# parklab/Salamander

Measured on AMD Instinct MI355X. Metric: KL-NMF update-steps/sec (96xN, k=50), higher is better.
Workload: dtype f64; 1 GPU; c2: KLNMF n_signatures=50 on synthetic Poisson counts 96x100000 per GPU (joint update_WH steps, device resident); n_features=96, n_samples_per_gpu=100000, n_samples_total=100000, n_signatures=50, parallelism=single GPU

## Files before the change

salamander_amd/csrc/salnmf_fused_kernel.h:

```cpp
#pragma once
#include "salnmf_kernels.h"

namespace salnmf {

constexpr int FK_NSEC = 16;
template <int KS, int KTM, int KR, bool DO_G, bool DO_U, bool DO_STATS, bool WTS = false, bool PERSIST = false, bool BLOCKED = false, bool RGIVEN = false,
          bool MVJ = false>
__global__ void __launch_bounds__(BLOCK, 1) fused_kernel(FusedParams p) {
#ifdef SALNMF_DEV_PROFILE
    unsigned long long tks[FK_NSEC] = {0, 0, 0, 0, 0, 0, 0, 0, 0, 0, 0, 0, 0, 0, 0, 0}, tk0 = __builtin_amdgcn_s_memtime(), tk1, ntl = 0;
#define FK_TICK(i) do { __builtin_amdgcn_sched_barrier(0); tk1 = __builtin_amdgcn_s_memtime(); tks[i] += tk1 - tk0; tk0 = tk1; __builtin_amdgcn_sched_barrier(0); } while (0)
#else
#define FK_TICK(i) do { } while (0)
#endif
    static_assert(!MVJ || (DO_G && DO_U && DO_STATS && !WTS && !PERSIST && !BLOCKED && !RGIVEN), "MVJ: the unweighted MvNMF pass pair");
    static_assert(!RGIVEN || (WTS && !DO_STATS && !PERSIST), "given ratio: the weighted-capable plain passes only (with BLOCKED: the update_H pass of one feature block)");
    static_assert(!PERSIST || (DO_G && DO_U && !DO_STATS && !WTS), "the persistent mode is the plain joint step");
    static_assert(!BLOCKED || (DO_U && !DO_STATS && WTS && !PERSIST), "feature blocks: the weighted-capable update_H pass, alone or with the block's numerator");
    using G_ = Geo<KS>;
    constexpr int KT = KTM;
    constexpr int KP = G_::KP, LS = G_::LS, HV = G_::HV;
    constexpr int KB = 16 * KTM;
    constexpr int NVP = KR == 0 ? 0 : (KR == 1 ? 4 : (KR == 2 ? 8 : 16));
    static_assert(KR >= 0 && KR <= 4 && KB + KR <= KP, "remainder columns must fit the padded layout");
    constexpr int WROWS = 4 * KS > 16 * KTM + KR ? 4 * KS : 16 * KTM + KR;
    static_assert(WROWS <= G_::WROWS, "never more rows than the padded layout");
    constexpr bool HDMA_FITS = (WROWS * WS + WAVES * (2 * G_::HL + G_::RL) + KP + (DO_STATS ? LOGTAB_DOUBLES : 0) + (WTS ? WAVES * 32 : 0)) * 8 <= 160 * 1024;
    constexpr bool HDMA = DO_G && DO_U && !PERSIST && !BLOCKED && !RGIVEN && !MVJ && HDMA_FITS;
    constexpr int REGION = (HDMA ? 2 : 1) * G_::HL + G_::RL;
    constexpr int LDSD = WROWS * WS + WAVES * REGION;
    constexpr int LDS_EXTRA = KP + (DO_STATS ? LOGTAB_DOUBLES : 0) + (WTS ? WAVES * 32 : 0);
    using CO_ = EpiGeo<KT, KR, 160 * 1024 / 8 - LDS_EXTRA>;
    constexpr int LDS_MAIN = LDSD > CO_::need(CO_::ROUNDS) ? LDSD : CO_::need(CO_::ROUNDS);
    __shared__ __attribute__((aligned(16))) double lds[LDS_MAIN + LDS_EXTRA];

    constexpr bool MVU = DO_U && DO_STATS && (!DO_G || MVJ);
    if (DO_STATS && p.skip_flag != nullptr && __hip_atomic_load((gsync_t*)p.skip_flag, __ATOMIC_RELAXED, __HIP_MEMORY_SCOPE_AGENT) != 0u) return;
    const int nwg = (int)gridDim.x - ((MVU && p.sideW != nullptr) ? 1 : 0);
    if (MVU && p.sideW != nullptr && (int)blockIdx.x == nwg) {
        static_assert(!MVU || KP * (MV_WS + 2 * MV_LD + 1) + 1 <= LDSD, "the W-only algebra must fit this geometry's LDS");
        const int K = p.K;
        double* Wl = lds;
        double* S = Wl + K * MV_WS;
        double* T = S + K * MV_LD;
        mv_prepare_W_body<BLOCK>(p.sideW, K, p.V, p.sideDelta, p.sideA, p.sideB, p.sideLogdet, Wl, S, T, T + K * MV_LD);
        return;
    }
    const int nsteps = PERSIST ? p.nsteps : 1;
    for (int step = 0; step < nsteps; ++step) {
    int tid = threadIdx.x;
    if (PERSIST) asm volatile("" : "+v"(tid));
    const int lane = tid & 63;
    const int wave = tid >> 6;
    const int c16 = lane & 15;
    const int q = lane >> 4;
    const int V = p.V, K = p.K;
    const int64_t N = p.N;
    const double* __restrict__ const wkl = WTS ? p.wkl : nullptr;
    const double* __restrict__ const wlh = WTS ? p.wlh : nullptr;

    double* Wl = lds;
    double* Hl = lds + WROWS * WS + wave * REGION;
    double* const Rl = lds + WROWS * WS + wave * REGION + G_::HL;
    double* Hnx = Hl + (HDMA ? G_::HL + G_::RL : 0);
    double* const Hdma0 = lds + WROWS * WS + __builtin_amdgcn_readfirstlane(wave) * REGION;
    int hsel = 0;

    double* hsl = lds + LDS_MAIN;
    if (p.hscale && tid < KP) hsl[tid] = p.hscale[tid];
    double* ltab = hsl + KP;
    if (DO_STATS) stage_logtab(ltab, tid);
    double* wgt = ltab + (DO_STATS ? LOGTAB_DOUBLES : 0) + wave * 32;

    d4 g[KT][VT];
    double grem[KR > 0 ? KR : 1][VT];
    double hsum[KT > 0 ? KT : 1];
    double hsum_rem = 0.0;
    double klacc = 0.0;
    double klacc_b = 0.0;
    if (MVU) {
#pragma unroll
        for (int kt = 0; kt < KT; ++kt) hsum[kt] = 0.0;
    }

    const int64_t tstride = (int64_t)(MVU ? nwg : (int)gridDim.x) * WAVES;
    int64_t tile = 0;
    constexpr bool COOP = DO_G && DO_U && !RGIVEN && !MVJ && !BLOCKED;
    constexpr int CSLAB = WROWS * WS + REGION;
    static_assert(!COOP || CO_::COOP_DOUBLES <= (WAVES - 1) * REGION, "the cooperative tile's numerator park must fit the idle waves' LDS");
    const int64_t nleft = p.ntiles % tstride;
    const bool coop = COOP && nleft > 0 && nleft <= (int64_t)gridDim.x && p.hscale == nullptr;
    const int64_t nfull = coop ? p.ntiles - nleft : p.ntiles;

    int hrow[HV], hcol[HV];
#pragma unroll
    for (int j = 0; j < HV; ++j) {
        int e = 2 * lane + 128 * j;
        hrow[j] = e / KP;
        hcol[j] = e - hrow[j] * KP;
    }

    d2 hpre[HV];
    double x[VT][4];
    d2 wpre = (d2){1.0, 0.0};

    constexpr int HPR = LS / 2, HNI = (16 * HPR + 63) / 64;
    int hoff[HDMA ? HNI : 1];
    if (HDMA) {
#pragma unroll
        for (int i = 0; i < HNI; ++i) {
            const int sp = 64 * i + lane, row = sp / HPR, c = sp - row * HPR;
            hoff[i] = row < 16 ? row * KP + 2 * (c < HPR - 1 ? c : HPR - 2) : -1;
        }
    }
    auto load_tile_H = [&](int64_t t) __attribute__((always_inline)) {
        const int64_t n0 = t * 16;
        if constexpr (HDMA) {
            const double* hsrc = p.H + n0 * KP;
            const unsigned m0base = (unsigned)(size_t)(__attribute__((address_space(3))) void*)(Hdma0 + hsel * (G_::HL + G_::RL));
#pragma unroll
            for (int i = 0; i < HNI; ++i)
                if (64 * (i + 1) <= 16 * HPR || hoff[i] >= 0)
                    asm volatile("s_mov_b32 m0, %1\n\ts_nop 0\n\tglobal_load_lds_dwordx4 %0, off"
                                 :
                                 : "v"(hsrc + hoff[i]), "s"(__builtin_amdgcn_readfirstlane(m0base + 1024u * i))
                                 : "memory");
            hsel ^= 1;
        } else {
            const d2* hsrc = reinterpret_cast<const d2*>(p.H + n0 * KP) + lane;
#pragma unroll
            for (int j = 0; j < HV; ++j) hpre[j] = hsrc[64 * j];
        }
    };
    auto load_tile_X = [&](int64_t t) __attribute__((always_inline)) {
        const int64_t n0 = t * 16;
        const double* xsrc = p.X + (n0 + q) * VMAX + c16;
#pragma unroll
        for (int vt = 0; vt < VT; ++vt)
#pragma unroll
            for (int r = 0; r < 4; ++r) x[vt][r] = xsrc[4 * r * VMAX + 16 * vt];
        if (WTS) {
            wpre[0] = p.wkl_eff[n0 + c16];
            wpre[1] = p.wlh_eff[n0 + c16];
        }
    };
    auto load_tile = [&](int64_t t) __attribute__((always_inline)) {
        load_tile_H(t);
        load_tile_X(t);
    };
    bool x_first = false;
    const bool coop_here = COOP && HDMA && coop && (int64_t)blockIdx.x < nleft;
    bool coop_fetched = false;
    auto coop_prefetch = [&]() __attribute__((always_inline)) {
        const int64_t ct = nfull + blockIdx.x;
        const int wvu = __builtin_amdgcn_readfirstlane(wave);
        if (wvu == 0) load_tile_H(ct);
        const int vt0 = wvu < 2 ? 2 * wvu : wvu + 2, nvt = wvu < 2 ? 2 : 1;
        const double* xsrc = p.X + (ct * 16 + q) * VMAX + c16;
#pragma unroll
        for (int i = 0; i < 2; ++i)
#pragma unroll
            for (int r = 0; r < 4; ++r) x[i][r] = xsrc[4 * r * VMAX + 16 * (vt0 + (i < nvt ? i : 0))];
        coop_fetched = true;
    };

    auto process_half = [&](int64_t tile, auto halftag) __attribute__((always_inline)) {
        constexpr int HALF = decltype(halftag)::value;
        constexpr bool TG = DO_G && HALF != 1, TU = DO_U && HALF != 2;
        const int64_t n0 = tile * 16;
        if (WTS) *reinterpret_cast<d2*>(wgt + 2 * c16) = wpre;
        if (!HDMA && HALF != 2 && p.hscale) {
#pragma unroll
            for (int j = 0; j < HV; ++j) {
                hpre[j][0] = clip_lo(hpre[j][0] * hsl[hcol[j]], kEps);
                hpre[j][1] = clip_lo(hpre[j][1] * hsl[hcol[j] + 1], kEps);
            }
        }
        if (!HDMA && HALF != 2) {
#pragma unroll
            for (int j = 0; j < HV; ++j) {
                *reinterpret_cast<d2*>(Hl + hrow[j] * LS + hcol[j]) = hpre[j];
            }
        }
        if (HDMA) {
            static_assert(VT * 4 == 24, "the X tile is 24 loads per lane");
            if (x_first) asm volatile("s_waitcnt vmcnt(0)" ::: "memory");
            else asm volatile("s_waitcnt vmcnt(24)" ::: "memory");
            x_first = false;
        }
        __builtin_amdgcn_wave_barrier();
        d4 uacc0[BLOCKED ? KT : 1];
        if (BLOCKED && TU) {
            const double* ua = p.Uacc + (n0 + q) * KP + c16;
#pragma unroll
            for (int kt = 0; kt < KT; ++kt)
#pragma unroll
                for (int r = 0; r < 4; ++r) uacc0[kt][r] = p.ublock != 1 ? ua[4 * r * KP + 16 * kt] : 0.0;
        }
        double uarem0 = 0.0;
        if (BLOCKED && TU && KR > 0 && p.ublock != 1) {
            const int ridx = NVP == 16 ? c16 : (NVP == 8 ? (c16 >> 1) : (c16 >> 2));
            const int jr0 = ridx >> 2, rr0 = ridx & 3;
            if (jr0 < KR && (c16 & (NVP == 16 ? 0 : (NVP == 8 ? 1 : 3))) == 0) uarem0 = p.Uacc[(n0 + q + 4 * rr0) * KP + KB + jr0];
        }
        constexpr int FKB = 1 + 7 * (HALF == 2 ? 1 : 0);
        FK_TICK(FKB + 0);

        double cv[4] = {0.0, 0.0, 0.0, 0.0};
        if (DO_STATS && (TG || p.KLpart != nullptr)) {
#pragma unroll
            for (int r = 0; r < 4; ++r) cv[r] = p.xlx[(n0 + q + 4 * r) * 16 + c16];
        }
        d4 pr[VT];
#pragma unroll
        for (int vt = 0; vt < VT; ++vt) pr[vt] = (d4){0, 0, 0, 0};
        if (RGIVEN) {
#pragma unroll
            for (int vt = 0; vt < VT; ++vt)
#pragma unroll
                for (int r = 0; r < 4; ++r) pr[vt][r] = x[vt][r];
        } else {
            const double* ha = Hl + c16 * LS + q;
            const double* wb = Wl + q * WS + c16;
            double a[2], b[2][VT];
            a[0] = ha[0];
#pragma unroll
            for (int vt = 0; vt < VT; ++vt) b[0][vt] = wb[16 * vt];
#pragma unroll
            for (int s = 0; s < KS; ++s) {
                __builtin_amdgcn_sched_barrier(0);
                if (s + 1 < KS) {
                    a[(s + 1) & 1] = ha[4 * (s + 1)];
#pragma unroll
                    for (int vt = 0; vt < VT; ++vt) b[(s + 1) & 1][vt] = wb[4 * (s + 1) * WS + 16 * vt];
                }
#pragma unroll
                for (int vt = 0; vt < VT; ++vt) pr[vt] = mfma(a[s & 1], b[s & 1][vt], pr[vt]);
#pragma unroll
                for (int vt = 0; vt < VT; ++vt) {
                    __builtin_amdgcn_sched_group_barrier(0x008, 1, 0);
                    __builtin_amdgcn_sched_group_barrier(0x100, 1, 0);
                }
                __builtin_amdgcn_sched_barrier(0);
            }
        }

        FK_TICK(FKB + 1);
        constexpr bool JKL = TG && TU && DO_STATS;
        if (JKL) {
            const double none[4] = {0.0, 0.0, 0.0, 0.0};
            klacc += tile_kl<false, (KR >= 3 ? 2 : 3)>(x, pr, none, cv, ltab, n0, N, V, q, c16);
        }
        double ga[4][KT];
        if (TG) {
#pragma unroll
            for (int r = 0; r < 4; ++r) {
                const double* ha = Hl + (4 * r + q) * LS + c16;
#pragma unroll
                for (int kt = 0; kt < KT; ++kt) ga[r][kt] = ha[16 * kt];
            }
        }

        if (DO_STATS && !JKL && (TG || p.KLpart != nullptr)) {
            const double none[4] = {0.0, 0.0, 0.0, 0.0};
            (HALF == 2 ? klacc_b : klacc) += tile_kl<false>(x, pr, none, cv, ltab, n0, N, V, q, c16);
        }
        FK_TICK(FKB + 2);
#pragma unroll
        for (int r = 0; r < (RGIVEN ? 0 : 4); ++r) {
            double rc[VT], t0[VT], t1[VT];
#pragma unroll
            for (int vt = 0; vt < VT; ++vt) rc[vt] = __builtin_amdgcn_rcp(pr[vt][r]);
#pragma unroll
            for (int vt = 0; vt < VT; ++vt) t0[vt] = __builtin_fma(-pr[vt][r], rc[vt], 1.0);
#pragma unroll
            for (int vt = 0; vt < VT; ++vt) rc[vt] = __builtin_fma(rc[vt], t0[vt], rc[vt]);
#pragma unroll
            for (int vt = 0; vt < VT; ++vt) t1[vt] = x[vt][r] * rc[vt];
#pragma unroll
            for (int vt = 0; vt < VT; ++vt) t0[vt] = __builtin_fma(-pr[vt][r], t1[vt], x[vt][r]);
#pragma unroll
            for (int vt = 0; vt < VT; ++vt) pr[vt][r] = __builtin_fma(t0[vt], rc[vt], t1[vt]);
        }
        asm volatile("" : "+v"(pr[0][0]), "+v"(pr[0][1]), "+v"(pr[0][2]), "+v"(pr[0][3]), "+v"(pr[1][0]), "+v"(pr[1][1]), "+v"(pr[1][2]),
                     "+v"(pr[1][3]), "+v"(pr[2][0]), "+v"(pr[2][1]), "+v"(pr[2][2]), "+v"(pr[2][3]), "+v"(pr[3][0]), "+v"(pr[3][1]));
        asm volatile("" : "+v"(pr[3][2]), "+v"(pr[3][3]), "+v"(pr[4][0]), "+v"(pr[4][1]), "+v"(pr[4][2]), "+v"(pr[4][3]), "+v"(pr[5][0]),
                     "+v"(pr[5][1]), "+v"(pr[5][2]), "+v"(pr[5][3]));

        FK_TICK(FKB + 3);
        if (HALF != 1 && tile + tstride < nfull) load_tile(tile + tstride);
        else if (HALF != 1 && coop_here) coop_prefetch();

        if (TU) {
#pragma unroll
            for (int vt = 0; vt < VT; ++vt)
#pragma unroll
                for (int r = 0; r < 4; ++r) Rl[(q + 4 * r) * RS + 16 * vt + c16] = pr[vt][r];
        }

        FK_TICK(FKB + 4);
        if (TG) {
            if (wkl) {
#pragma unroll
                for (int r = 0; r < 4; ++r) {
                    double wk = wgt[2 * (q + 4 * r)];
#pragma unroll
                    for (int kt = 0; kt < KT; ++kt) ga[r][kt] *= wk;
                }
            }
#pragma unroll
            for (int r = 0; r < 4; ++r)
#pragma unroll
                for (int kt = 0; kt < KT; ++kt)
#pragma unroll
                    for (int vt = 0; vt < VT; ++vt) mfma_agpr(g[kt][vt], ga[r][kt], pr[vt][r]);
            if (KR > 0) {
#pragma unroll
                for (int r = 0; r < 4; ++r) {
                    double wk = wkl ? wgt[2 * (q + 4 * r)] : 1.0;
#pragma unroll
                    for (int j = 0; j < KR; ++j) {
                        double hv = Hl[(4 * r + q) * LS + KB + j];
                        if (wkl) hv *= wk;
#pragma unroll
                        for (int vt = 0; vt < VT; ++vt) grem[j][vt] = __builtin_fma(hv, pr[vt][r], grem[j][vt]);
                    }
                }
            }
        }
        double urem[NVP > 0 ? NVP : 1];
        if (TU && KR > 0) {
#pragma unroll
            for (int i = 0; i < NVP; ++i) urem[i] = 0.0;
            double wj[KR > 0 ? KR : 1][VT];
#pragma unroll
            for (int j = 0; j < KR; ++j)
#pragma unroll
                for (int vt = 0; vt < VT; ++vt) wj[j][vt] = Wl[(KB + j) * WS + 16 * vt + c16];
#pragma unroll
            for (int vt = 0; vt < VT; ++vt)
#pragma unroll
                for (int j = 0; j < KR; ++j)
#pragma unroll
                    for (int r = 0; r < 4; ++r) urem[4 * j + r] = __builtin_fma(pr[vt][r], wj[j][vt], urem[4 * j + r]);
        }
        __builtin_amdgcn_wave_barrier();
        FK_TICK(FKB + 5);
#ifdef SALNMF_DEV_PROFILE
        if (HALF != 1) ++ntl;
#endif

        if (TU) {
            d4 u[KT];
#pragma unroll
            for (int kt = 0; kt < KT; ++kt) u[kt] = BLOCKED ? uacc0[kt] : (d4){0, 0, 0, 0};
            double hcur[4][KT];
#pragma unroll
            for (int r = 0; r < 4; ++r)
#pragma unroll
                for (int kt = 0; kt < KT; ++kt) hcur[r][kt] = Hl[(q + 4 * r) * LS + 16 * kt + c16];
            auto rs_stage = [&](auto mtag, auto livetag) __attribute__((always_inline)) {
                constexpr int M = decltype(mtag)::value, LIVE = decltype(livetag)::value;
                if (LIVE > 1) {
                    constexpr int half = LIVE / 2;
                    const bool upper = (c16 & M) != 0;
#pragma unroll
                    for (int i = 0; i < half; ++i) {
                        double send = upper ? urem[i] : urem[i + half];
                        double keep = upper ? urem[i + half] : urem[i];
                        urem[i] = keep + xor16<M>(send);
                    }
                } else {
                    urem[0] += xor16<M>(urem[0]);
                }
            };
            const int rs_idx = NVP == 16 ? c16 : (NVP == 8 ? (c16 >> 1) : (c16 >> 2));
            const double* ra = Rl + c16 * RS + q;
            const double* wb = Wl + c16 * WS + q;
            double a[2], b[2][KT];
            a[0] = ra[0];
#pragma unroll
            for (int kt = 0; kt < KT; ++kt) b[0][kt] = wb[16 * kt * WS];
#pragma unroll
            for (int s = 0; s < VSTEPS; ++s) {
                __builtin_amdgcn_sched_barrier(0);
                if (s + 1 < VSTEPS) {
                    a[(s + 1) & 1] = ra[4 * (s + 1)];
#pragma unroll
                    for (int kt = 0; kt < KT; ++kt) b[(s + 1) & 1][kt] = wb[16 * kt * WS + 4 * (s + 1)];
                }
#pragma unroll
                for (int kt = 0; kt < KT; ++kt) u[kt] = mfma(a[s & 1], b[s & 1][kt], u[kt]);
#pragma unroll
                for (int kt = 0; kt < KT; ++kt) {
                    __builtin_amdgcn_sched_group_barrier(0x008, 1, 0);
                    __builtin_amdgcn_sched_group_barrier(0x100, 2, 0);
                }
                __builtin_amdgcn_sched_barrier(0);
            }
            if (KR > 0) { using std::integral_constant; rs_stage(integral_constant<int, 8>{}, integral_constant<int, NVP>{}); rs_stage(integral_constant<int, 4>{}, integral_constant<int, (NVP / 2 > 1 ? NVP / 2 : 1)>{}); rs_stage(integral_constant<int, 2>{}, integral_constant<int, (NVP / 4 > 1 ? NVP / 4 : 1)>{}); rs_stage(integral_constant<int, 1>{}, integral_constant<int, (NVP / 8 > 1 ? NVP / 8 : 1)>{}); }
            if (BLOCKED) {
                double* ua = p.Uacc + (n0 + q) * KP + c16;
                const int jr = rs_idx >> 2, rr = rs_idx & 3;
                const bool rem_owner = KR > 0 && jr < KR && (c16 & (NVP == 16 ? 0 : (NVP == 8 ? 1 : 3))) == 0;
                double* uar = p.Uacc + (n0 + q + 4 * rr) * KP + KB + jr;
                if (KR > 0 && rem_owner) urem[0] += uarem0;
                if (p.ublock != 3) {
#pragma unroll
                    for (int r = 0; r < 4; ++r)
#pragma unroll
                        for (int kt = 0; kt < KT; ++kt) ua[4 * r * KP + 16 * kt] = u[kt][r];
                    if (KR > 0 && rem_owner) *uar = urem[0];
                    FK_TICK(FKB + 6);
                    return;
                }
            }
            double* hdst = p.Hout + (n0 + q) * KP + c16;
            if (wlh == nullptr) {
#pragma unroll
                for (int r = 0; r < 4; ++r)
#pragma unroll
                    for (int kt = 0; kt < KT; ++kt) {
                        const double hn = clip_lo(hcur[r][kt] * u[kt][r], p.hfloor);
                        __builtin_nontemporal_store(hn, &hdst[4 * r * KP + 16 * kt]);
                        if (HALF == 1) Hl[(q + 4 * r) * LS + 16 * kt + c16] = hn;
                        if (MVU) hsum[kt] += (n0 + q + 4 * r < N) ? hn : 0.0;
                    }
            } else {
#pragma unroll
                for (int r = 0; r < 4; ++r) {
                    const int64_t n = n0 + q + 4 * r;
                    const double wl = wgt[2 * (q + 4 * r) + 1];
                    double wk2 = 1.0;
                    if (wkl) { double w = wgt[2 * (q + 4 * r)]; wk2 = w * w; }
#pragma unroll
                    for (int kt = 0; kt < KT; ++kt) {
                        double inter = 4.0 * hcur[r][kt] * u[kt][r];
                        if (wkl) inter *= wk2;
                        double disc = 0.25 * wl * wl + inter;
                        double t = wl / 2 - sqrt(disc);
                        double hn = 0.25 * (t * t);
                        if (wkl) hn /= wk2;
                        hn = clip_lo(hn, kEps);
                        __builtin_nontemporal_store(hn, &hdst[4 * r * KP + 16 * kt]);
                        if (MVU) hsum[kt] += (n < N) ? hn : 0.0;
                    }
                }
            }
            if (KR > 0) {
                const int j = rs_idx >> 2, r = rs_idx & 3;
                const int lowmask = NVP == 16 ? 0 : (NVP == 8 ? 1 : 3);
                if (j < KR && (c16 & lowmask) == 0) {
                    const int64_t n = n0 + q + 4 * r;
                    const double h = Hl[(q + 4 * r) * LS + KB + j];
                    double hn;
                    if (wlh == nullptr) {
                        hn = h * urem[0];
                    } else {
                        const double wl = wgt[2 * (q + 4 * r) + 1];
                        double wk2 = 1.0;
                        if (wkl) { double w = wgt[2 * (q + 4 * r)]; wk2 = w * w; }
                        double inter = 4.0 * h * urem[0];
                        if (wkl) inter *= wk2;
                        double disc = 0.25 * wl * wl + inter;
                        double t = wl / 2 - sqrt(disc);
                        hn = 0.25 * (t * t);
                        if (wkl) hn /= wk2;
                    }
                    hn = clip_lo(hn, p.hfloor);
                    p.Hout[n * KP + KB + j] = hn;
                    if (HALF == 1) Hl[(q + 4 * r) * LS + KB + j] = hn;
                    if (MVU) hsum_rem += (n < N) ? hn : 0.0;
                }
            }
        }
        FK_TICK(FKB + 6);
    };

    if (DO_G) {
#pragma unroll
        for (int kt = 0; kt < KT; ++kt)
#pragma unroll
            for (int vt = 0; vt < VT; ++vt) g[kt][vt] = (d4){0, 0, 0, 0};
        if (KR > 0) {
#pragma unroll
            for (int j = 0; j < KR; ++j)
#pragma unroll
                for (int vt = 0; vt < VT; ++vt) grem[j][vt] = 0.0;
        }
    }
    auto process_tile_coop = [&](int64_t ctile) __attribute__((always_inline)) {
        const int64_t n0 = ctile * 16;
        int tid = threadIdx.x;
        asm volatile("" : "+v"(tid));
        const int lane = tid & 63, wave = tid >> 6, c16 = lane & 15, q = lane >> 4;
        const bool pre = HDMA && coop_fetched;
        double* Hs = lds + WROWS * WS + ((pre && ((nfull / tstride) & 1)) ? G_::HL + G_::RL : 0);
        double* cslab = lds + CSLAB;
        double* Rs = lds + WROWS * WS + G_::HL;
        const int wv = __builtin_amdgcn_readfirstlane(wave);
        constexpr int HR = (16 * KP + 2 * BLOCK - 1) / (2 * BLOCK);
        d2 hst[HR];
        const int vt0 = wv < 2 ? 2 * wv : wv + 2, nvt = wv < 2 ? 2 : 1;
        double xx[2][4];
        if (pre) {
#pragma unroll
            for (int i = 0; i < 2; ++i)
#pragma unroll
                for (int r = 0; r < 4; ++r) xx[i][r] = x[i][r];
        } else {
#pragma unroll
            for (int j = 0; j < HR; ++j) {
                const int e = 2 * tid + 2 * BLOCK * j;
                hst[j] = (e < 16 * KP) ? *reinterpret_cast<const d2*>(p.H + n0 * KP + e) : (d2){0, 0};
            }
            const double* xsrc = p.X + (n0 + q) * VMAX + c16;
#pragma unroll
            for (int i = 0; i < 2; ++i)
#pragma unroll
                for (int r = 0; r < 4; ++r) xx[i][r] = (i < nvt) ? xsrc[4 * r * VMAX + 16 * (vt0 + i)] : 0.0;
        }
        double* wg0 = ltab + (DO_STATS ? LOGTAB_DOUBLES : 0);
        d2 wco = (d2){1.0, 0.0};
        if (WTS && tid < 16) {
            wco[0] = p.wkl_eff[n0 + tid];
            wco[1] = p.wlh_eff[n0 + tid];
        }
        if (pre) asm volatile("s_waitcnt vmcnt(0)" ::: "memory");
        __syncthreads();
        if (WTS && tid < 16) *reinterpret_cast<d2*>(wg0 + 2 * tid) = wco;
        if (!pre) {
#pragma unroll
            for (int j = 0; j < HR; ++j) {
                const int e = 2 * tid + 2 * BLOCK * j;
                if (e < 16 * KP) {
                    const int row = e / KP, col = e - row * KP;
                    *reinterpret_cast<d2*>(Hs + row * LS + col) = hst[j];
                }
            }
        }
        if (WTS || !pre) __syncthreads();
        FK_TICK(9);
        auto phase_a = [&](auto vtag, const double (&xv)[4]) __attribute__((always_inline)) {
            constexpr int VTI = decltype(vtag)::value;
            d4 pp = (d4){0, 0, 0, 0};
            const double* ha = Hs + c16 * LS + q;
            const double* wb = Wl + q * WS + 16 * VTI + c16;
#pragma unroll
            for (int s2 = 0; s2 < KS; ++s2) pp = mfma(ha[4 * s2], wb[4 * s2 * WS], pp);
            if (DO_STATS) {
                bool valid[4], ok = true;
#pragma unroll
                for (int r = 0; r < 4; ++r) {
                    valid[r] = (n0 + q + 4 * r < N) && (16 * VTI + c16 < V);
                    ok &= !valid[r] || log_pos_ok(pp[r]);
                }
                if (VTI == 0) {
#pragma unroll
                    for (int r = 0; r < 4; ++r) klacc += p.xlx[(n0 + q + 4 * r) * 16 + c16];
                }
                if (__all(ok)) {
                    double ps[4], lp[4];
#pragma unroll
                    for (int r = 0; r < 4; ++r) ps[r] = valid[r] ? pp[r] : 1.0;
                    log_pos_n<4>(ps, ltab, lp);
#pragma unroll
                    for (int r = 0; r < 4; ++r) klacc += valid[r] ? __builtin_fma(-xv[r], lp[r], ps[r]) : 0.0;
                } else {
#pragma unroll
                    for (int r = 0; r < 4; ++r)
                        if (valid[r]) klacc += kl_term_p(xv[r], pp[r]);
                }
            }
#pragma unroll
            for (int r = 0; r < 4; ++r) {
                pp[r] = div_path(xv[r], pp[r]);
                Rs[(q + 4 * r) * RS + 16 * VTI + c16] = pp[r];
            }
            d4 gc[KT];
#pragma unroll
            for (int kt = 0; kt < KT; ++kt) gc[kt] = (d4){0, 0, 0, 0};
#pragma unroll
            for (int r = 0; r < 4; ++r)
#pragma unroll
                for (int kt = 0; kt < KT; ++kt) {
                    double ha = Hs[(4 * r + q) * LS + 16 * kt + c16];
                    if (WTS && wkl) ha *= wg0[2 * (4 * r + q)];
                    gc[kt] = mfma(ha, pp[r], gc[kt]);
                }
#pragma unroll
            for (int kt = 0; kt < KT; ++kt)
#pragma unroll
                for (int r2 = 0; r2 < 4; ++r2) cslab[((kt * VT + VTI) * 4 + r2) * 64 + lane] = gc[kt][r2];
            if (KR > 0) {
#pragma unroll
                for (int j = 0; j < KR; ++j) {
                    double t = 0.0;
#pragma unroll
                    for (int r = 0; r < 4; ++r) {
                        double hv = Hs[(4 * r + q) * LS + KB + j];
                        if (WTS && wkl) hv *= wg0[2 * (4 * r + q)];
                        t = __builtin_fma(hv, pp[r], t);
                    }
                    t = rows_sum(t);
                    if (q == 0) cslab[CO_::COOP_REM + j * VMAX + 16 * VTI + c16] = t;
                }
            }
        };
        {
            using std::integral_constant;
            if (wv == 0) { phase_a(integral_constant<int, 0>{}, xx[0]); phase_a(integral_constant<int, 1>{}, xx[1]); }
            else if (wv == 1) { phase_a(integral_constant<int, 2>{}, xx[0]); phase_a(integral_constant<int, 3>{}, xx[1]); }
            else if (wv == 2) phase_a(integral_constant<int, 4>{}, xx[0]);
            else phase_a(integral_constant<int, 5>{}, xx[0]);
        }
        __syncthreads();
        FK_TICK(10);
        if (wv < KT) {
            const int kt = wv;
            d4 u = (d4){0, 0, 0, 0};
            const double* ra = Rs + c16 * RS + q;
            const double* wb = Wl + (16 * kt + c16) * WS + q;
#pragma unroll
            for (int s2 = 0; s2 < VSTEPS; ++s2) u = mfma(ra[4 * s2], wb[4 * s2], u);
            double* hdst = p.Hout + (n0 + q) * KP + 16 * kt + c16;
#pragma unroll
            for (int r = 0; r < 4; ++r) {
                const double h = Hs[(q + 4 * r) * LS + 16 * kt + c16];
                double hn = h * u[r];
                if (WTS && wlh) hn = lhalf_update(h, u[r], wg0[2 * (q + 4 * r) + 1], wkl ? wg0[2 * (q + 4 * r)] : 1.0, wkl != nullptr);
                __builtin_nontemporal_store(clip_lo(hn, WTS && wlh ? kEps : p.hfloor), &hdst[4 * r * KP]);
            }
        } else if (KR > 0 && wv == KT) {
            const int n = lane & 15, j = lane >> 4;
            if (j < KR) {
                const double* rr = Rs + n * RS;
                const double* wr = Wl + (KB + j) * WS;
                double dot = 0.0;
                for (int v = 0; v < VMAX; ++v) dot = __builtin_fma(rr[v], wr[v], dot);
                const double h = Hs[n * LS + KB + j];
                double hn = h * dot;
                if (WTS && wlh) hn = lhalf_update(h, dot, wg0[2 * n + 1], wkl ? wg0[2 * n] : 1.0, wkl != nullptr);
                p.Hout[(n0 + n) * KP + KB + j] = clip_lo(hn, WTS && wlh ? kEps : p.hfloor);
            }
        }
    };

    tile = (int64_t)blockIdx.x * WAVES + wave;
    if (PERSIST) {
        if (tile < nfull) load_tile(tile);
        if (step > 0 && !persist_wait_W(p.sync, p.abort_host, (unsigned)step * (unsigned)K, lds, tid)) return;
        stage_W<WROWS, true>(Wl, p.Wmut, K, V, V, tid);
        __syncthreads();
    } else {
        if (p.wdma && V == VMAX && p.ldw == VMAX && (reinterpret_cast<uintptr_t>(p.W) & 15) == 0) {
            stage_W_dma_issue<WROWS>(Wl, p.W, K, tid);
            asm volatile("s_waitcnt vmcnt(0) lgkmcnt(0)" ::: "memory");
            __builtin_amdgcn_s_barrier();
            asm volatile("" ::: "memory");
            if (tile < nfull) load_tile(tile);
        } else {
            stage_W<WROWS>(Wl, p.W, K, V, p.ldw, tid);
            __syncthreads();
            if (tile < nfull) {
                if (HDMA) {
                    load_tile_X(tile);
                    load_tile_H(tile);
                    x_first = true;
                } else {
                    load_tile(tile);
                }
            }
        }
    }
    FK_TICK(0);
    for (; tile < nfull; tile += tstride) {
        using std::integral_constant;
        if constexpr (MVJ) {
            process_half(tile, integral_constant<int, 1>{});
            process_half(tile, integral_constant<int, 2>{});
        } else {
            process_half(tile, integral_constant<int, 0>{});
        }
        if (HDMA) {
            double* t = Hl;
            Hl = Hnx;
            Hnx = t;
        }
    }
    FK_TICK(8);
    if (COOP && coop && (int64_t)blockIdx.x < nleft) process_tile_coop(nfull + blockIdx.x);
    FK_TICK(12);

    __syncthreads();
    FK_TICK(11);
    if (DO_G) {
        asm volatile("s_nop 15\n\ts_nop 7" ::: "memory");
#pragma unroll
        for (int kt = 0; kt < KT; ++kt)
#pragma unroll
            for (int vt = 0; vt < VT; ++vt) asm volatile("" : "+a"(g[kt][vt]));
        constexpr int ROUNDS = CO_::ROUNDS, VTR = CO_::VTR, NT = CO_::NT, MAXI = CO_::MAXI;
        double* remL = lds + CO_::PARK;
        const int wv = __builtin_amdgcn_readfirstlane(wave);
        const bool coopwg = COOP && coop && (int64_t)blockIdx.x < nleft;
        double cc[ROUNDS][MAXI][4];
        double crem[2] = {0.0, 0.0};
        if (COOP && coopwg) {
            const double* cl = lds + CSLAB;
#pragma unroll
            for (int half = 0; half < ROUNDS; ++half)
#pragma unroll
                for (int i = 0; i < MAXI; ++i) {
                    const int t = wv + WAVES * i < NT ? wv + WAVES * i : NT - 1;
                    const int kt = t / VTR, vt = half * VTR + (t - kt * VTR);
#pragma unroll
                    for (int r = 0; r < 4; ++r) cc[half][i][r] = cl[((kt * VT + vt) * 4 + r) * 64 + lane];
                }
            if (KR > 0) {
#pragma unroll
                for (int it = 0; it < 2; ++it) {
                    const int i = tid + it * BLOCK;
                    crem[it] = cl[CO_::COOP_REM + (i < KR * VMAX ? i : 0)];
                }
            }
            __syncthreads();
        }
        double* out = p.Gpart + (int64_t)blockIdx.x * K * VMAX;
#pragma unroll
        for (int half = 0; half < ROUNDS; ++half) {
            double* mine = lds + (size_t)wv * NT * 256 + lane;
#pragma unroll
            for (int kt = 0; kt < KT; ++kt)
#pragma unroll
                for (int h = 0; h < VTR; ++h)
#pragma unroll
                    for (int r = 0; r < 4; ++r) mine[((kt * VTR + h) * 4 + r) * 64] = g[kt][half * VTR + h][r];
            if (KR > 0 && half == 0) {
#pragma unroll
                for (int j = 0; j < KR; ++j)
#pragma unroll
                    for (int vt = 0; vt < VT; ++vt) {
                        const double t = rows_sum(grem[j][vt]);
                        if (q == 0) remL[(wv * KR + j) * VMAX + 16 * vt + c16] = t;
                    }
            }
            __syncthreads();
            FK_TICK(13);
#pragma unroll
            for (int i = 0; i < MAXI; ++i) {
                const int t = wv + WAVES * i;
                if (t < NT) {
                    const int kt = t / VTR, vt = half * VTR + (t - kt * VTR);
                    const double* from = lds + (size_t)t * 256 + lane;
                    double acc[4];
#pragma unroll
                    for (int r = 0; r < 4; ++r) {
                        acc[r] = from[r * 64];
#pragma unroll
                        for (int w = 1; w < WAVES; ++w) acc[r] += from[(size_t)w * NT * 256 + r * 64];
                    }
                    if (COOP && coopwg) {
#pragma unroll
                        for (int r = 0; r < 4; ++r) acc[r] += cc[half][i][r];
                    }
                    const int v = 16 * vt + c16;
#pragma unroll
                    for (int r = 0; r < 4; ++r) {
                        const int k = 16 * kt + q + 4 * r;
                        if (k < K && v < V) st_shared<PERSIST>(&out[k * VMAX + v], acc[r]);
                    }
                }
            }
            if (KR > 0 && half == 0) {
#pragma unroll
                for (int it = 0; it < 2; ++it) {
                    const int i = tid + it * BLOCK;
                    if (i < KR * VMAX) {
                        const int j = i / VMAX, v = i - j * VMAX;
                        double t = ((remL[j * VMAX + v] + remL[(KR + j) * VMAX + v]) + remL[(2 * KR + j) * VMAX + v]) + remL[(3 * KR + j) * VMAX + v];
                        if (COOP && coopwg) t += crem[it];
                        if (v < V) st_shared<PERSIST>(&out[(KB + j) * VMAX + v], t);
                    }
                }
            }
            if (half + 1 < ROUNDS) __syncthreads();
        }
        FK_TICK(14);
    }
    if (PERSIST) {
        if (!persist_publish_and_tail(p.sync, p.abort_host, p.Gpart, p.G, p.Wmut, K, V, p.n_given, lds, step, tid)) return;
    }
    if (MVU) {
        __syncthreads();
        double* S = lds;
#pragma unroll
        for (int kt = 0; kt < KT; ++kt) S[(16 * kt + c16) * 16 + wave * 4 + q] = hsum[kt];
        if (KR > 0) {
            const int idx = NVP == 16 ? c16 : (NVP == 8 ? (c16 >> 1) : (c16 >> 2));
            const int lowmask = NVP == 16 ? 0 : (NVP == 8 ? 1 : 3);
            const int j = idx >> 2;
            for (int jj = 0; jj < KR; ++jj) {
                double v = (j == jj && (c16 & lowmask) == 0) ? hsum_rem : 0.0;
#pragma unroll
                for (int m = 1; m < 16; m <<= 1) v += __shfl_xor(v, m, 64);
                if (c16 == 0) S[(KB + jj) * 16 + wave * 4 + q] = v;
            }
        }
        __syncthreads();
        if (tid < K) {
            double t = 0.0;
            for (int i = 0; i < 16; ++i) t += S[tid * 16 + i];
            p.Hsumpart[(int64_t)blockIdx.x * K + tid] = t;
        }
    }
    if (MVJ) {
        __syncthreads();
        double* Kb = lds;
        Kb[tid] = klacc_b;
        __syncthreads();
        for (int h = BLOCK / 2; h > 0; h >>= 1) {
            if (tid < h) Kb[tid] += Kb[tid + h];
            __syncthreads();
        }
        if (tid == 0) p.KLpartB[blockIdx.x] = Kb[0];
    }
    if (DO_STATS && ((DO_G && !MVJ) || p.KLpart != nullptr)) {
        __syncthreads();
        double* Ks = lds;
        Ks[tid] = klacc;
        __syncthreads();
        for (int h = BLOCK / 2; h > 0; h >>= 1) {
            if (tid < h) Ks[tid] += Ks[tid + h];
            __syncthreads();
        }
        if (!(MVU && p.kl_out != nullptr)) {
            if (tid == 0) p.KLpart[blockIdx.x] = Ks[0];
        } else {
            if (tid == 0) {
                __hip_atomic_store((gdouble*)(p.KLpart + blockIdx.x), Ks[0], __ATOMIC_RELAXED, __HIP_MEMORY_SCOPE_AGENT);
                asm volatile("s_waitcnt vmcnt(0)" ::: "memory");
                const unsigned ticket = __hip_atomic_fetch_add((gsync_t*)p.kl_counter, 1u, __ATOMIC_RELAXED, __HIP_MEMORY_SCOPE_AGENT);
                Ks[1] = (ticket == (unsigned)nwg - 1u) ? 1.0 : 0.0;
            }
            __syncthreads();
            const bool last = Ks[1] != 0.0;
            __syncthreads();
            if (last) {
                __builtin_amdgcn_fence(__ATOMIC_ACQUIRE, "wavefront");
                double sum = 0.0;
                for (int i = tid; i < nwg; i += BLOCK) sum += ld_shared<true>(p.KLpart + i);
                Ks[tid] = sum;
                __syncthreads();
                for (int h = BLOCK / 2; h > 0; h >>= 1) {
                    if (tid < h) Ks[tid] += Ks[tid + h];
                    __syncthreads();
                }
                if (tid == 0) {
                    p.kl_out[0] = Ks[0];
                    __hip_atomic_store((gsync_t*)p.kl_counter, 0u, __ATOMIC_RELAXED, __HIP_MEMORY_SCOPE_AGENT);
                }
            }
        }
    }
    }
    FK_TICK(15);
#ifdef SALNMF_DEV_PROFILE
    if (p.prof != nullptr && (threadIdx.x & 63) == 0) {
        unsigned long long* row = p.prof + ((size_t)blockIdx.x * WAVES + (threadIdx.x >> 6)) * (FK_NSEC + 1);
        for (int i = 0; i < FK_NSEC; ++i) row[i] += tks[i];
        row[FK_NSEC] += ntl;
    }
#endif
#undef FK_TICK
}

}
```

Baseline: 14580 update-steps/s.

## Rebalance phase-A work across waves and vectorize remainder-column H update

Splits the per-tile phase into a ratio stage and a gradient stage. Waves 2 and 3, which have only one V tile, now also compute the gradient for that tile before the barrier, and afterwards pick up the gradient for a tile produced by waves 0 and 1, reading its ratio from LDS. This is meant to even out per-wave work. The remainder-column H update replaces a serial per-lane dot-product loop over VMAX with register FMAs followed by a cross-lane xor reduce-scatter. Per-sample weights are now staged into a per-wave LDS slot, which removes one barrier; this adds LDS traffic and register pressure, and the weighted update is open-coded inline.

```diff
diff --git a/salamander_amd/csrc/salnmf_fused_kernel.h b/salamander_amd/csrc/salnmf_fused_kernel.h
--- a/salamander_amd/csrc/salnmf_fused_kernel.h
+++ b/salamander_amd/csrc/salnmf_fused_kernel.h
@@ -520,15 +520,15 @@
 #pragma unroll
                 for (int r = 0; r < 4; ++r) xx[i][r] = (i < nvt) ? xsrc[4 * r * VMAX + 16 * (vt0 + i)] : 0.0;
         }
-        double* wg0 = ltab + (DO_STATS ? LOGTAB_DOUBLES : 0);
-        d2 wco = (d2){1.0, 0.0};
-        if (WTS && tid < 16) {
-            wco[0] = p.wkl_eff[n0 + tid];
-            wco[1] = p.wlh_eff[n0 + tid];
+        double* wg0 = ltab + (DO_STATS ? LOGTAB_DOUBLES : 0) + wv * 32;
+        if (WTS) {
+            d2 wco;
+            wco[0] = p.wkl_eff[n0 + c16];
+            wco[1] = p.wlh_eff[n0 + c16];
+            *reinterpret_cast<d2*>(wg0 + 2 * c16) = wco;
         }
         if (pre) asm volatile("s_waitcnt vmcnt(0)" ::: "memory");
         __syncthreads();
-        if (WTS && tid < 16) *reinterpret_cast<d2*>(wg0 + 2 * tid) = wco;
         if (!pre) {
 #pragma unroll
             for (int j = 0; j < HR; ++j) {
@@ -539,11 +539,11 @@
                 }
             }
         }
-        if (WTS || !pre) __syncthreads();
+        if (!pre) __syncthreads();
         FK_TICK(9);
-        auto phase_a = [&](auto vtag, const double (&xv)[4]) __attribute__((always_inline)) {
+        auto phase_p = [&](auto vtag, const double (&xv)[4], d4& pp) __attribute__((always_inline)) {
             constexpr int VTI = decltype(vtag)::value;
-            d4 pp = (d4){0, 0, 0, 0};
+            pp = (d4){0, 0, 0, 0};
             const double* ha = Hs + c16 * LS + q;
             const double* wb = Wl + q * WS + 16 * VTI + c16;
 #pragma unroll
@@ -577,6 +577,9 @@
                 pp[r] = div_path(xv[r], pp[r]);
                 Rs[(q + 4 * r) * RS + 16 * VTI + c16] = pp[r];
             }
+        };
+        auto phase_g = [&](auto vtag, const d4& pp) __attribute__((always_inline)) {
+            constexpr int VTI = decltype(vtag)::value;
             d4 gc[KT];
 #pragma unroll
             for (int kt = 0; kt < KT; ++kt) gc[kt] = (d4){0, 0, 0, 0};
@@ -607,15 +610,25 @@
                 }
             }
         };
-        {
-            using std::integral_constant;
-            if (wv == 0) { phase_a(integral_constant<int, 0>{}, xx[0]); phase_a(integral_constant<int, 1>{}, xx[1]); }
-            else if (wv == 1) { phase_a(integral_constant<int, 2>{}, xx[0]); phase_a(integral_constant<int, 3>{}, xx[1]); }
-            else if (wv == 2) phase_a(integral_constant<int, 4>{}, xx[0]);
-            else phase_a(integral_constant<int, 5>{}, xx[0]);
-        }
+        auto shared_r = [&](auto vtag) __attribute__((always_inline)) {
+            constexpr int VTI = decltype(vtag)::value;
+            d4 t;
+#pragma unroll
+            for (int r = 0; r < 4; ++r) t[r] = Rs[(q + 4 * r) * RS + 16 * VTI + c16];
+            return t;
+        };
+        using std::integral_constant;
+        d4 r0 = (d4){0, 0, 0, 0}, r1 = (d4){0, 0, 0, 0};
+        if (wv == 0) { phase_p(integral_constant<int, 0>{}, xx[0], r0); phase_p(integral_constant<int, 1>{}, xx[1], r1); }
+        else if (wv == 1) { phase_p(integral_constant<int, 2>{}, xx[0], r0); phase_p(integral_constant<int, 3>{}, xx[1], r1); }
+        else if (wv == 2) { phase_p(integral_constant<int, 4>{}, xx[0], r0); phase_g(integral_constant<int, 4>{}, r0); }
+        else { phase_p(integral_constant<int, 5>{}, xx[0], r0); phase_g(integral_constant<int, 5>{}, r0); }
         __syncthreads();
         FK_TICK(10);
+        if (wv == 0) phase_g(integral_constant<int, 0>{}, r0);
+        else if (wv == 1) phase_g(integral_constant<int, 2>{}, r0);
+        else if (wv == 2) phase_g(integral_constant<int, 1>{}, shared_r(integral_constant<int, 1>{}));
+        else phase_g(integral_constant<int, 3>{}, shared_r(integral_constant<int, 3>{}));
         if (wv < KT) {
             const int kt = wv;
             d4 u = (d4){0, 0, 0, 0};
@@ -632,16 +645,64 @@
                 __builtin_nontemporal_store(clip_lo(hn, WTS && wlh ? kEps : p.hfloor), &hdst[4 * r * KP]);
             }
         } else if (KR > 0 && wv == KT) {
-            const int n = lane & 15, j = lane >> 4;
-            if (j < KR) {
-                const double* rr = Rs + n * RS;
-                const double* wr = Wl + (KB + j) * WS;
-                double dot = 0.0;
-                for (int v = 0; v < VMAX; ++v) dot = __builtin_fma(rr[v], wr[v], dot);
-                const double h = Hs[n * LS + KB + j];
-                double hn = h * dot;
-                if (WTS && wlh) hn = lhalf_update(h, dot, wg0[2 * n + 1], wkl ? wg0[2 * n] : 1.0, wkl != nullptr);
-                p.Hout[(n0 + n) * KP + KB + j] = clip_lo(hn, WTS && wlh ? kEps : p.hfloor);
+            double pr[VT][4], wj[KR > 0 ? KR : 1][VT], urem[NVP > 0 ? NVP : 1];
+#pragma unroll
+            for (int vt = 0; vt < VT; ++vt)
+#pragma unroll
+                for (int r = 0; r < 4; ++r) pr[vt][r] = Rs[(q + 4 * r) * RS + 16 * vt + c16];
+#pragma unroll
+            for (int j = 0; j < KR; ++j)
+#pragma unroll
+                for (int vt = 0; vt < VT; ++vt) wj[j][vt] = Wl[(KB + j) * WS + 16 * vt + c16];
+#pragma unroll
+            for (int i = 0; i < NVP; ++i) urem[i] = 0.0;
+#pragma unroll
+            for (int vt = 0; vt < VT; ++vt)
+#pragma unroll
+                for (int j = 0; j < KR; ++j)
+#pragma unroll
+                    for (int r = 0; r < 4; ++r) urem[4 * j + r] = __builtin_fma(pr[vt][r], wj[j][vt], urem[4 * j + r]);
+            auto rs_stage = [&](auto mtag, auto livetag) __attribute__((always_inline)) {
+                constexpr int M = decltype(mtag)::value, LIVE = decltype(livetag)::value;
+                if (LIVE > 1) {
+                    constexpr int half = LIVE / 2;
+                    const bool upper = (c16 & M) != 0;
+#pragma unroll
+                    for (int i = 0; i < half; ++i) {
+                        double send = upper ? urem[i] : urem[i + half];
+                        double keep = upper ? urem[i + half] : urem[i];
+                        urem[i] = keep + xor16<M>(send);
+                    }
+                } else {
+                    urem[0] += xor16<M>(urem[0]);
+                }
+            };
+            rs_stage(integral_constant<int, 8>{}, integral_constant<int, NVP>{});
+            rs_stage(integral_constant<int, 4>{}, integral_constant<int, (NVP / 2 > 1 ? NVP / 2 : 1)>{});
+            rs_stage(integral_constant<int, 2>{}, integral_constant<int, (NVP / 4 > 1 ? NVP / 4 : 1)>{});
+            rs_stage(integral_constant<int, 1>{}, integral_constant<int, (NVP / 8 > 1 ? NVP / 8 : 1)>{});
+            const int rs_idx = NVP == 16 ? c16 : (NVP == 8 ? (c16 >> 1) : (c16 >> 2));
+            const int j = rs_idx >> 2, r = rs_idx & 3;
+            const int lowmask = NVP == 16 ? 0 : (NVP == 8 ? 1 : 3);
+            if (j < KR && (c16 & lowmask) == 0) {
+                const int64_t n = n0 + q + 4 * r;
+                const double h = Hs[(q + 4 * r) * LS + KB + j];
+                double hn;
+                if (wlh == nullptr) {
+                    hn = h * urem[0];
+                } else {
+                    const double wl = wg0[2 * (q + 4 * r) + 1];
+                    double wk2 = 1.0;
+                    if (wkl) { double w = wg0[2 * (q + 4 * r)]; wk2 = w * w; }
+                    double inter = 4.0 * h * urem[0];
+                    if (wkl) inter *= wk2;
+                    double disc = 0.25 * wl * wl + inter;
+                    double t = wl / 2 - sqrt(disc);
+                    hn = 0.25 * (t * t);
+                    if (wkl) hn /= wk2;
+                }
+                hn = clip_lo(hn, p.hfloor);
+                p.Hout[n * KP + KB + j] = hn;
             }
         }
     };
```

Result: no change. 14590 update-steps/s, median of 3 (+0.1%).
